# xiph/daala

Measured on NVIDIA H100. Metric: encoder Mpixels/s on 4K YUV420 intra, higher is better.
Workload: dtype int32

## Files before the change

### daala_b200/csrc/kf_engine.cu

```cuda
#include <cuda_runtime.h>
#include <math.h>
#include <stdint.h>
#include <stdio.h>
#include <stdlib.h>
#include <string.h>

#include <algorithm>
#include <cmath>
#include <mutex>
#include <new>
#include <vector>

#include "daala_b200.h"
#include "dering_search.h"
#include "late_skip.h"
#include "mc_batch.h"
#include "gen/coding_order.inc"
#include "pvq_math.cuh"
#include "pvq_warp.cuh"
#include "pvq_common.cuh"

namespace daala_b200 {
namespace kf {

// ... 679 lines not shown
    reinterpret_cast<short4*>(S.res_pack)[r] = pk;
  }
}

struct ItemGeom {
  int blk, band, bn, q, beta, pli, qoff;
  size_t off;
};
__device__ __forceinline__ int band_q(const daala_b200_pvq_params& prm, const daala_b200_kf_frame_quant* fq, int frame,
                                      int pli, int qidx) {
  return fq ? (fq[frame].q0 * fq[frame].pvq_qm_q4[pli][qidx]) >> 4 : (prm.q0 * prm.pvq_qm_q4[pli][qidx]) >> 4;
}
__device__ __forceinline__ ItemGeom item_geom(const daala_b200_pvq_params& prm, uint32_t item,
                                              const daala_b200_kf_frame_quant* fq) {
  ItemGeom g;
  g.blk = (int)(item >> 4);
  g.band = (int)(item & 15);
  const daala_b200_pvq_block b = prm.blocks[g.blk];
  const int bs = b.bs;
  g.pli = b.pli;
  const int start = band_start(g.band);
  g.bn = band_start(g.band + 1) - start;
  g.off = (size_t)b.coef_off + start;
  const int qidx = bs * (bs + 1) + (g.band + 1) - (g.band + 1) / 3;
  int q = band_q(prm, fq, b.frame, g.pli, qidx);
  g.q = q < 1 ? 1 : q;
  g.beta = (prm.use_masking && g.pli == 0 && bs > 0) ? kBeta15 : kBeta1;
  g.qoff = (b.xdec & 1 ? prm.qm_stride : 0) + ((((1 << (2 * bs)) - 1) << 4) / 3) + start;
  return g;
}

template <int kPhase, bool kZeroRef, int kMode, bool kFq = false>
__global__ void __launch_bounds__(128) k_pvq_split(const __grid_constant__ Stage S, int cls, int chunk) {
  const daala_b200_pvq_params& prm = S.prm;
  const int lane = threadIdx.x & 31;
  const int slots = S.sp_slots[cls];
  const int first = chunk * slots;
  const int count = min(S.cnt[S.n_items_at + cls] - first, slots);
  const int vs = cls == 2 ? 128 : 32;
  const int nwarps = (gridDim.x * blockDim.x) >> 5;
  for (int i = (blockIdx.x * blockDim.x + threadIdx.x) >> 5; i < count; i += nwarps) {
    const ItemGeom g = item_geom(prm, S.items[cls][first + i], kFq ? S.fq : nullptr);
    int16_t* vec = S.sp_vec[cls] + (size_t)i * 3 * vs;
    int32_t* lanes = S.sp_lanes[cls] + (size_t)i * kCtxLaneWords * 16;
    int32_t* uni = S.sp_uni[cls] + (size_t)i * kCtxUniWords;
    int16_t* snap = S.sp_snap[cls] + (size_t)i * kMaxEvents * vs;
    const int32_t* r0 = kZeroRef ? nullptr : prm.ref + g.off;
    BandCtx B;
    if (kPhase == 0) {
      band_setup<kMode>(lane, B, prm.in + g.off, r0, g.bn, g.q, g.beta, prm.is_keyframe, g.pli, prm.qm + g.qoff,
                 prm.pvq_norm_lambda, S.rsqrt_tbl);
      band_ctx_store_setup(lane, B, g.bn, vec, vs, lanes, uni);
    } else if (kPhase == 1) {
      band_ctx_load_search(lane, B, g.bn, vec, vs, lanes);
      band_search<kMode>(lane, B, g.bn, snap, vs, S.rsqrt_tbl);
      band_ctx_store_search(lane, B, lanes);
    } else {
      band_ctx_load_finish(lane, B, g.bn, vec, vs, lanes, uni);
      int itheta, max_theta, k;
      double skip_term;
      const int gain = band_finish<kMode>(lane, B, snap, vs, prm.out + g.off, r0, g.bn, g.q, prm.y + g.off, &itheta, &max_theta, &k,
                                   g.beta, &skip_term, prm.is_keyframe, g.pli, prm.qm_inv + g.qoff, prm.pvq_norm_lambda);
      if (lane == 0) {
        const size_t r = (size_t)g.blk * 9 + g.band;
        prm.res_skip_term[r] = skip_term;
        short4 pk;
        pk.x = (short)gain; pk.y = (short)itheta; pk.z = (short)max_theta; pk.w = (short)k;
        reinterpret_cast<short4*>(S.res_pack)[r] = pk;
      }
    }
  }
}

template <int kMode>
// ... 1292 lines not shown
}

static int enqueue_dering_luma(daala_b200_kf* kf, const Dering& D, cudaStream_t s) {
  if (D.search) {
    const int rc = daala_b200_dering_search_enqueue(&D.sb, s);
    if (rc) return rc;
  }
  const int nsb = kf->nhsb * kf->nvsb;
  k_dering_thresholds<<<(kf->F * nsb + 255) / 256, 256, 0, s>>>(
      D.level, D.thr[0], D.thr[1], kf->F * nsb, make_int4(D.tbl[0][0], D.tbl[0][1], D.tbl[0][2], D.tbl[0][3]),
      make_int2(D.tbl[0][4], D.tbl[0][5]), make_int4(D.tbl[1][0], D.tbl[1][1], D.tbl[1][2], D.tbl[1][3]),
      make_int2(D.tbl[1][4], D.tbl[1][5]), D.coded, D.applied, D.frame_tbl, nsb);
  return enqueue_dering_plane(kf, D, 0, s);
}

static int enqueue_dering(daala_b200_kf* kf, const Dering& D, cudaStream_t s) {
  int rc = enqueue_recon(D.frame, 0, 3, s);
  if (!rc) rc = enqueue_dering_luma(kf, D, s);
  for (int p = 1; !rc && p < 3; p++) rc = enqueue_dering_plane(kf, D, p, s);
  return rc;
}

static int dering_launches(const Dering& D, int parts) { return 2 * parts + (D.search ? 5 + 6 + 6 + 1 : 0) + 1 + 3; }

template <bool kZeroRef, bool kFq = false>
static void enqueue_split(daala_b200_kf* kf, const Stage& S, cudaStream_t s) {
  const int grid = kf->sms * 16;
  for (int cls = 2; cls >= 0; cls--) {
    for (int chunk = 0; chunk < S.sp_chunks[cls]; chunk++) {
      if (cls == 2) {
        k_pvq_split<0, kZeroRef, 2, kFq><<<grid, 128, 0, s>>>(S, cls, chunk);
        k_pvq_split<1, kZeroRef, 2><<<grid, 128, 0, s>>>(S, cls, chunk);
        k_pvq_split<2, kZeroRef, 2, kFq><<<grid, 128, 0, s>>>(S, cls, chunk);
      } else {
        k_pvq_split<0, kZeroRef, 1, kFq><<<grid, 128, 0, s>>>(S, cls, chunk);
        k_pvq_split<1, kZeroRef, 1><<<grid, 128, 0, s>>>(S, cls, chunk);
        k_pvq_split<2, kZeroRef, 1, kFq><<<grid, 128, 0, s>>>(S, cls, chunk);
      }
    }
  }
}

template <bool kInter>
static void enqueue_sym(const Sym& Y, int wide, cudaStream_t s) {
  k_sym_rank<<<(Y.F * Y.nsb + 7) / 8, 256, 0, s>>>(Y);
  k_sym_sb_scan<<<1, 1024, 0, s>>>(Y);
  k_sym_place<<<wide, 256, 0, s>>>(Y);
  k_sym_tile_sums<<<Y.ntiles, kTile, 0, s>>>(Y);
  k_sym_tile_scan<<<1, 1024, 0, s>>>(Y);
  k_sym_offsets<<<Y.ntiles, kTile, 0, s>>>(Y);
  k_sym_pack<kInter><<<wide, 256, 0, s>>>(Y);
  k_sym_index<<<1, 256, 0, s>>>(Y);
}

static int kf_enqueue_step_inter(daala_b200_kf* kf, int phases) {
  cudaStream_t s = kf->stream;
  const Lists& L = kf->lists;
  const int wide = kf->sms * 8;
  if (phases & DAALA_B200_KF_LISTS) {
    k_unit_tile_sums<<<L.ntiles, kTile, 0, s>>>(L);
    k_tile_scan<<<1, 1024, 0, s>>>(L);
    k_unit_emit<<<L.ntiles, kTile, 0, s>>>(L);
    k_luma_items<<<wide, 256, 0, s>>>(L);
    k_chroma_items<<<wide, 256, 0, s>>>(L);
    if (kf->cfg.inter_mc) {
      if (cudaMemsetAsync(L.cnt + kMcBadRef, 0, 2 * sizeof(int32_t), s) != cudaSuccess) return (int)cudaGetLastError();
// ... 837 lines not shown
```

### daala_b200/csrc/pvq_warp.cuh

```cuda
#pragma once
#include <math.h>
#include <stdint.h>

#include "pvq_math.cuh"

namespace daala_b200 {
namespace pvq {

constexpr unsigned kFull = 0xffffffffu;
constexpr int kMaxEvents = 14;
constexpr int kRsqrtEntries = 1 << 16;
constexpr int kLogEntries = 1 << 12;
constexpr int kTableDoubles = kRsqrtEntries + kLogEntries;

#ifndef DAALA_B200_PVQ_EXACT_BOUND
#define DAALA_B200_PVQ_EXACT_BOUND 4503599627370496.
#endif
#ifdef DAALA_B200_EMU_STATS
#define PVQ_WARP_STAT(i) (daala_b200_pvq_warp_stats[i]++)
#else
#define PVQ_WARP_STAT(i) ((void)0)
#endif

__device__ __forceinline__ int wsum(int v) { return __reduce_add_sync(kFull, v); }
__device__ __forceinline__ int wmax(int v) { return __reduce_max_sync(kFull, v); }
__device__ __forceinline__ int wmin(int v) { return __reduce_min_sync(kFull, v); }
__device__ __forceinline__ unsigned wmaxu(unsigned v) { return __reduce_max_sync(kFull, v); }
__device__ __forceinline__ long long wsum64(long long s) {
  const int lo = (int)(s & 0xffffff);
  const int hi = (int)(s >> 24);
  return ((long long)wsum(hi) << 24) + wsum(lo);
}
__device__ __forceinline__ double wfetch(double v, int src) {
  int lo = __double2loint(v), hi = __double2hiint(v);
  lo = __shfl_sync(kFull, lo, src);
  hi = __shfl_sync(kFull, hi, src);
  return __hiloint2double(hi, lo);
}
__device__ __forceinline__ int ordered_key(float f) {
  const int b = __float_as_int(f);
  return b ^ ((b >> 31) & 0x7fffffff);
}
__device__ __forceinline__ int pick4(const int (&a)[4], int slot) {
  int v = a[0];
#pragma unroll
  for (int e = 1; e < 4; e++) if (slot == e) v = a[e];
  return v;
}

static __device__ __noinline__ double nl_log(double x) { return log(x); }
static __device__ __noinline__ double nl_acos(double x) { return acos(x); }
static __device__ __noinline__ double nl_sqrt(double x) { return sqrt(x); }
static __device__ __noinline__ double nl_div(double a, double b) { return a / b; }
static __device__ __noinline__ int nl_cos(int32_t x) { return pvq_cos(x); }
static __device__ __noinline__ double nl_rsqrt_small(int i) {
  if (i <= 16) return kRsqrtSmall[i - 1];
  return 1. / sqrt((double)i);
}
__device__ __forceinline__ void pvq_fill_rsqrt_table(double* rsq, int i) {
  if (i < kRsqrtEntries) rsq[i] = i > 0 ? nl_rsqrt_small(i) : 0.;
  else rsq[i] = .9 * (M_LOG2E * nl_log((double)(i > kRsqrtEntries ? i - kRsqrtEntries : 1)));
}
static __device__ __noinline__ long long nl_gain(int32_t acc, int q0, int beta, int bshift) {
  int32_t g;
  const int32_t cg = compute_gain_from_energy(acc, q0, &g, beta, bshift);
  return ((long long)cg << 32) | (uint32_t)g;
}
static __device__ __noinline__ long long nl_theta_k(int32_t qcg, int j, int ts, int noref, int n, int beta) {
  const int32_t qtheta = noref ? 0 : compute_theta(j, ts);
  const int k = compute_k(qcg, j, noref, n, beta);
  return ((long long)qtheta << 32) | (uint32_t)k;
}

__device__ __forceinline__ void householder_apply_warp(int lane, bool big, int (&out)[4], const int (&x)[4],
                                                       const int (&r)[4], int n) {
  int32_t l2r = 0, proj = 0;
#pragma unroll
  for (int e = 0; e < 4; e++) {
    if (e && !big) break;
    if (e * 32 + lane < n) {
      l2r += mul16(r[e], r[e]);
      proj += mul16(r[e], x[e]);
    }
  }
  l2r = wsum(l2r);
  proj = wsum(proj);
  int l2r_shift = (ilog((uint32_t)l2r) - 1) - 14;
  int16_t l2r_norm = (int16_t)vshr_round(l2r, l2r_shift);
  int16_t rcp = rcp16(l2r_norm);
  int proj_shift = (ilog((uint32_t)abs(proj)) - 1) - 14;
  int16_t proj_norm = (int16_t)vshr_round(proj, proj_shift);
  int16_t proj_1 = (int16_t)mul16_q15(proj_norm, rcp);
  int outshift = 14 - proj_shift - 1 + l2r_shift;
  if (outshift > 30) outshift = 30;
#pragma unroll
  for (int e = 0; e < 4; e++) {
    if (e && !big) break;
    int32_t t = mul16(r[e], proj_1);
    t = outshift >= 0 ? shr_round(t, outshift) : shl(t, -outshift);
    out[e] = (int16_t)(x[e] - t);
  }
}

struct SearchVec {
  int xa[4];
  double xx, norm_1, l1_norm;
  double delta_rate;
  int xmax, nn;
};

template <int E>
__device__ __forceinline__ void search_init(int lane, SearchVec& v, const int (&src)[4], int nn) {
  long long sxx = 0;
  int xmax = 0, sl1 = 0;
#pragma unroll
  for (int e = 0; e < E; e++) {
    const int a = e * 32 + lane < nn ? abs(src[e]) : 0;
    v.xa[e] = a;
    sxx += (long long)a * a;
    sl1 += a;
    xmax = a > xmax ? a : xmax;
  }
  v.xx = (double)wsum64(sxx);
  v.xmax = wmax(xmax);
  v.l1_norm = (double)wsum(sl1);
  v.norm_1 = nl_div(1., nl_sqrt(1e-30 + v.xx));
  v.delta_rate = nl_div(3., (double)nn);
  v.nn = nn;
}

__device__ __forceinline__ int search_start(int lane, const SearchVec& v, int (&ya)[4], int k, int prev_k, bool big,
                                            double* xy, double* yy) {
  const int nn = v.nn;
  long long sxy = 0, syy = 0;
  int si = 0;
  if (prev_k > 0 && prev_k <= k) {
#pragma unroll
    for (int e = 0; e < 4; e++) {
      if (e && !big) break;
      if (e * 32 + lane >= nn) ya[e] = 0;
      sxy += (long long)v.xa[e] * ya[e];
      syy += (long long)ya[e] * ya[e];
      si += ya[e];
    }
  } else if (k > 2) {
    const double l1_inv = nl_div(1., v.l1_norm > 1e-100 ? v.l1_norm : 1e-100);
#pragma unroll
    for (int e = 0; e < 4; e++) {
      if (e && !big) break;
      const double tmp = k * (double)v.xa[e] * l1_inv;
      const int f = (int)floor(tmp);
      ya[e] = (e * 32 + lane < nn && f > 0) ? f : 0;
      sxy += (long long)v.xa[e] * ya[e];
      syy += (long long)ya[e] * ya[e];
      si += ya[e];
    }
  } else {
#pragma unroll
    for (int e = 0; e < 4; e++) ya[e] = 0;
    *xy = 0;
    *yy = 0;
    return 0;
  }
  *xy = (double)wsum64(sxy);
  *yy = (double)wsum64(syy);
  return wsum(si);
}

template <int E>
__device__ __forceinline__ void search_event(int lane, const SearchVec& v, int (&ya)[4], int k, int i, double xy,
                                             double yy, double lambda, const double* rsq, double* xy_out,
                                             double* yy_out) {
  const int nn = v.nn;
  const int rdo_pulses = 1 + k / 4;
  double delta_rate = v.delta_rate;
  double accel_rate = 0.;
  if (k == 1) {
    if (nn == 15) {
      accel_rate = -8. / 15;
      delta_rate = 4.5 / 15 - accel_rate;
    } else if (nn == 8) {
      accel_rate = 5.7 / 8;
      delta_rate = 9.3 / 8 - accel_rate;
    }
  }
  for (; i < k; i++) {
    const bool plain = i < k - rdo_pulses;
    bool cont[E];
    double tval[E];
    int total;
    if (plain) {
      const double bound = (xy + v.xmax) * (xy + v.xmax) * (yy + 2. * i + 1.);
      if (bound < DAALA_B200_PVQ_EXACT_BOUND) {
        const float xyf = (float)xy, yyf1 = (float)(yy + 1.);
        unsigned key[E], kmax = 0;
#pragma unroll
        for (int e = 0; e < E; e++) {
          float a = xyf + (float)v.xa[e];
          a *= a;
// ... 62 lines not shown
#pragma unroll
          for (int t = 1; t < E; t++) if (e == t) m = mk[t];
        }
        if (!m) break;
        const int l = __ffs(m) - 1;
        m &= m - 1;
        int sxa = v.xa[0], sya = ya[0];
        double stv = tval[0];
#pragma unroll
        for (int t = 1; t < E; t++) if (e == t) { sxa = v.xa[t]; sya = ya[t]; stv = tval[t]; }
        if (plain) {
          const int xj = __shfl_sync(kFull, sxa, l);
          const int yj = __shfl_sync(kFull, sya, l);
          double a = xy + (double)xj;
          const double b = yy + 2 * yj + 1;
          a *= a;
          if (pos < 0 || a * bb > ba * b) { ba = a; bb = b; pos = e * 32 + l; }
        } else {
          const double t = wfetch(stv, l);
          if (pos < 0 || t > ba) { ba = t; pos = e * 32 + l; }
        }
      }
    }
    const int src = pos & 31, slot = pos >> 5;
    int sx = v.xa[0], sy = ya[0];
#pragma unroll
    for (int e = 1; e < E; e++) if (slot == e) { sx = v.xa[e]; sy = ya[e]; }
    const int px = __shfl_sync(kFull, sx, src);
    const int py = __shfl_sync(kFull, sy, src);
    xy = xy + (double)px;
    yy = yy + 2 * py + 1;
#pragma unroll
    for (int e = 0; e < E; e++) if (e * 32 + lane == pos) ya[e]++;
  }
  *xy_out = xy;
  *yy_out = yy;
}

struct BandCtx {
  int x16[4], r16[4], xr[4];
  int32_t cg, g, gain_offset;
  int icgr, m, s;
  double best_dist, best_cost, skip_dist;
  int c_gain, c_theta, c_ts, c_k, c_cosd, c_alive, c_ev;
  int32_t c_qcg, c_qtheta;
  double c_sinprod, c_lambda, c_rate_ts;
  double e_xy, e_yy, e_xx;
  int e_sum, e_k, e_zero;
};

constexpr int kCtxLaneWords = 24;
constexpr int kCtxUniWords = 16;
constexpr int kSnapEntries = kMaxEvents * kMaxN + 3 * kMaxN + 2 * (kCtxLaneWords * 16 + kCtxUniWords);

#ifdef __CUDACC__
__device__ __forceinline__ void ctx_sync() { __syncwarp(); }
#else
inline void ctx_sync() {}
#endif

__device__ __forceinline__ void ctx_put_d(int32_t* lanes, int w, int lane, double v) {
  lanes[w * 16 + lane] = __double2loint(v);
  lanes[(w + 1) * 16 + lane] = __double2hiint(v);
}
__device__ __forceinline__ double ctx_get_d(const int32_t* lanes, int w, int lane) {
  return __hiloint2double(lanes[(w + 1) * 16 + lane], lanes[w * 16 + lane]);
// ... 78 lines not shown
  B.c_rate_ts = ctx_get_d(lanes, 12, l);
  B.c_ev = on ? lanes[14 * 16 + l] : -1;
  B.e_xy = on ? ctx_get_d(lanes, 15, l) : 0.;
  B.e_yy = on ? ctx_get_d(lanes, 17, l) : 0.;
  B.e_xx = on ? ctx_get_d(lanes, 19, l) : 0.;
  B.e_sum = on ? lanes[21 * 16 + l] : 0;
  B.e_k = on ? lanes[22 * 16 + l] : 0;
  B.e_zero = on ? lanes[23 * 16 + l] : 0;
  B.cg = uni[0]; B.g = uni[1]; B.gain_offset = uni[2]; B.icgr = uni[3]; B.m = uni[4]; B.s = uni[5];
  B.best_dist = __hiloint2double(uni[7], uni[6]);
  B.best_cost = __hiloint2double(uni[9], uni[8]);
  B.skip_dist = __hiloint2double(uni[11], uni[10]);
}

template <int kMode>
__device__ __forceinline__ void band_setup(int lane, BandCtx& B, const int32_t* x0, const int32_t* r0, int n, int q0,
                                           int beta, int is_keyframe, int pli, const int16_t* qm,
                                           double pvq_norm_lambda, const double* rsq) {
  int (&x16)[4] = B.x16; int (&r16)[4] = B.r16; int (&xr)[4] = B.xr;
  int32_t &cg = B.cg, &g = B.g, &gain_offset = B.gain_offset;
  int &icgr = B.icgr, &m = B.m, &s = B.s;
  double &best_dist = B.best_dist, &best_cost = B.best_cost, &skip_dist = B.skip_dist;
  int &c_gain = B.c_gain, &c_theta = B.c_theta, &c_ts = B.c_ts, &c_k = B.c_k, &c_cosd = B.c_cosd, &c_alive = B.c_alive;
  int32_t &c_qcg = B.c_qcg, &c_qtheta = B.c_qtheta;
  double &c_sinprod = B.c_sinprod, &c_lambda = B.c_lambda, &c_rate_ts = B.c_rate_ts;

  const double gain_weight = 1.4;
  const double cgain_1 = 1. / kCgainOne;
  const double cgain_2 = cgain_1 * cgain_1;
  const double theta_scale = (1 << kThetaShift) * 2. / M_PI;
  const double theta_scale_1 = 1. / theta_scale;
  const double trig_1 = 1. / 32768;
  const bool big = kMode == 0 ? n > 32 : kMode == 2;
  int xshift, rshift, r_nonnull = 0;
  {
    int32_t xv[4], rv[4];
    int32_t sx = 0, sr = 0;
#pragma unroll
    for (int e = 0; e < 4; e++) {
      xv[e] = rv[e] = 0;
      if (e && !big) continue;
      const int j = e * 32 + lane;
      if (j < n) {
        xv[e] = x0[j];
        rv[e] = r0 ? r0[j] : 0;
      }
      const int16_t tx = (int16_t)(xv[e] >> 8), tr = (int16_t)(rv[e] >> 8);
      sx += tx * (int32_t)tx;
      sr += tr * (int32_t)tr;
      r_nonnull |= rv[e] != 0;
    }
    sx = wsum(sx);
    sr = wsum(sr);
    r_nonnull = __any_sync(kFull, r_nonnull);
    xshift = 9 + ilog((uint32_t)(n + sx)) / 2 - 15;
    rshift = 9 + ilog((uint32_t)(n + sr)) / 2 - 14;
    if (xshift < 0) xshift = 0;
    if (rshift < 0) rshift = 0;
#pragma unroll
    for (int e = 0; e < 4; e++) {
      x16[e] = r16[e] = xr[e] = 0;
      if (e && !big) continue;
      const int j = e * 32 + lane;
      const int qmv = j < n ? qm[j] : 0;
      x16[e] = (int16_t)shr_round(xv[e] * qmv, kQmShift + xshift);
      r16[e] = (int16_t)shr_round(rv[e] * qmv, kQmShift + rshift);
    }
  }
  long long scorr = 0;
  int32_t accx = 0, accr = 0;
#pragma unroll
  for (int e = 0; e < 4; e++) {
    if (e && !big) break;
    scorr += mul16(x16[e], r16[e]);
    accx += x16[e] * x16[e];
    accr += r16[e] * r16[e];
  }
  double corr = (double)wsum64(scorr);
  accx = wsum(accx);
  accr = wsum(accr);
  int32_t gr, cgr;
  {
    const long long pk = nl_gain(lane & 1 ? accr : accx, q0, beta, lane & 1 ? rshift : xshift);
    const int gl = (int)(uint32_t)pk, cgl = (int)(pk >> 32);
    g = __shfl_sync(kFull, gl, 0);
    cg = __shfl_sync(kFull, cgl, 0);
    gr = __shfl_sync(kFull, gl, 1);
    cgr = __shfl_sync(kFull, cgl, 1);
  }
  const int cfl_enabled = is_keyframe && pli != 0;
  if (cfl_enabled) cgr = kCgainOne;
  icgr = shr_round(cgr, kCgainShift);
  gain_offset = cgr - shl(icgr, kCgainShift);
  best_dist = gain_weight * cg * cg * cgain_2;
  best_cost = best_dist + pvq_norm_lambda * 0.;
  corr = nl_div(corr, 1e-100 + nl_div(g * (double)gr, (double)shl(1, xshift + rshift)));
  corr = corr < 1. ? corr : 1.;
  corr = corr > -1. ? corr : -1.;
  if (is_keyframe) {
    skip_dist = gain_weight * cg * cg * cgain_2;
  } else {
    skip_dist = gain_weight * (cg - cgr) * (cg - cgr) + cgr * (double)cg * (2 - 2 * corr);
    skip_dist *= cgain_2;
    const int32_t scgr = gain_offset > 0 ? gain_offset : 0;
    if (icgr == 0) {
      best_dist = gain_weight * (cg - scgr) * (cg - scgr) + scgr * (double)cg * (2 - 2 * corr);
      best_dist *= cgain_2;
    }
    best_cost = best_dist + pvq_norm_lambda * 0.;
  }
  const double dist0 = best_dist;

  const bool have_ref = r_nonnull && corr > 0;
  int32_t theta = 0;
  m = 0;
  s = 1;
  if (have_ref) {
    theta = round32(theta_scale * nl_acos(corr));
    int key = -1;
#pragma unroll
    for (int e = 0; e < 4; e++) {
      if (e && !big) break;
      const int j = e * 32 + lane;
      const int kk = j < n ? (abs(r16[e]) << 7) | (127 - j) : -1;
      key = kk > key ? kk : key;
    }
    key = wmax(key);
    m = (key >> 7) > 0 ? 127 - (key & 127) : 0;
    const int rm = __shfl_sync(kFull, pick4(r16, m >> 5), m & 31);
    s = rm > 0 ? 1 : -1;
#pragma unroll
    for (int e = 0; e < 4; e++)
      if (e * 32 + lane == m) r16[e] = (int16_t)(r16[e] + shr_round(gr * s, rshift));
    householder_apply_warp(lane, big, xr, x16, r16, n);
#pragma unroll
    for (int e = 0; e < 4; e++) {
      if (e && !big) break;
      const int t1 = __shfl_sync(kFull, xr[e], (lane + 1) & 31);
      const int t2 = e + 1 < 4 ? __shfl_sync(kFull, xr[e + 1 < 4 ? e + 1 : e], 0) : 0;
      const int nxt = lane == 31 ? t2 : t1;
      if (e * 32 + lane >= m) xr[e] = nxt;
    }
  }

  c_gain = 0; c_theta = -1; c_ts = 0; c_k = 0; c_cosd = 0; c_qcg = 0; c_qtheta = 0;
  c_sinprod = 0; c_lambda = 0; c_rate_ts = 0;
  bool c_valid = false;
  {
    const bool wref = lane < 12;
    const bool nref = lane == 12 || lane == 13;
    int i = 0, j = -1;
    if (wref && have_ref) {
      const int gain_bound = (cg - gain_offset) >> kCgainShift;
      i = (gain_bound - 1 > 1 ? gain_bound - 1 : 1) + (lane >> 2);
      c_valid = i <= gain_bound + 1;
      c_qcg = shl(i, kCgainShift) + gain_offset;
    } else if (nref && ((is_keyframe && pli == 0) || corr < .5 || cg < (int32_t)shl(2, kCgainShift))) {
      const int gain_bound = cg >> kCgainShift;
      i = (gain_bound > 1 ? gain_bound : 1) + (lane - 12);
      c_valid = i <= gain_bound + 1;
      c_qcg = shl(i, kCgainShift);
    }
    if (!c_valid) c_qcg = kCgainOne;
    if (wref) {
      c_ts = compute_max_theta(c_qcg, beta);
      int lo = (int)floor(.5 + nl_div(theta * theta_scale_1 * 2, M_PI) * c_ts) - 2;
      int hi = (int)ceil(nl_div(theta * theta_scale_1 * 2, M_PI) * c_ts);
      if (lo < 0) lo = 0;
      if (hi > c_ts - 1) hi = c_ts - 1;
      j = lo + (lane & 3);
// ... 1 lines not shown
    } else {
      c_ts = 0;
    }
    const long long tk = nl_theta_k(c_qcg, j, c_ts, !wref, n, beta);
    c_qtheta = (int32_t)(tk >> 32);
    c_k = (int)(uint32_t)tk;
    c_gain = i;
    c_theta = wref ? j : -1;
    c_cosd = nl_cos(theta - c_qtheta);
    const int sin_q = nl_cos(32768 - c_qtheta), sin_t = nl_cos(32768 - theta);
    double dist = gain_weight * (c_qcg - cg) * (c_qcg - cg);
    double g2 = c_qcg * (double)cg;
    if (wref) {
      const double dist_theta = 2 - 2. * c_cosd * trig_1;
      dist = dist + c_qcg * (double)cg * dist_theta;
      const double sin_theta = sin_t * trig_1;
      c_sinprod = sin_theta * sin_q * trig_1;
      g2 = g2 * c_sinprod;
    }
    dist *= cgain_2;
    g2 = g2 * cgain_2;
    c_alive = c_valid && !(wref ? dist > dist0 + 1.0 * pvq_norm_lambda && c_k != 0 : dist > dist0 && c_k != 0);
    c_lambda = nl_div(pvq_norm_lambda, 1e-30 + g2);
    c_rate_ts = c_ts < kLogEntries ? rsq[kRsqrtEntries + (c_ts > 0 ? c_ts : 1)]
                                   : .9 * (M_LOG2E * nl_log((double)c_ts));
  }
}

template <int kMode>
__device__ __forceinline__ void band_search(int lane, BandCtx& B, int n, int16_t* snap, int snap_stride,
                                            const double* rsq, const int32_t* pre_ev = nullptr,
                                            const int16_t* pre_snap = nullptr) {
  const bool big = kMode == 0 ? n > 32 : kMode == 2;
  const int (&x16)[4] = B.x16; const int (&xr)[4] = B.xr;
  const int &c_k = B.c_k, &c_alive = B.c_alive;
  const double &c_lambda = B.c_lambda;
  int &c_ev = B.c_ev;
  double &e_xy = B.e_xy, &e_yy = B.e_yy, &e_xx = B.e_xx;
  int &e_sum = B.e_sum, &e_k = B.e_k, &e_zero = B.e_zero;
  unsigned alive_w = __ballot_sync(kFull, c_alive && lane < 12);
  unsigned alive_n = __ballot_sync(kFull, c_alive && lane >= 12);
  if (pre_ev) alive_n = 0;

  int ya[4];
#pragma unroll
  for (int e = 0; e < 4; e++) ya[e] = 0;
  SearchVec sv;
  sv.nn = n;
  sv.xx = 0;
  int prev_k = 0, nev = 0;
  c_ev = -1;
  int phase = 0;
  e_xy = 0; e_yy = 0; e_xx = 0; e_sum = 0; e_k = 0; e_zero = 0;
  while (alive_w | alive_n) {
    unsigned grp;
    int kcur, leader;
    const bool noref_ev = alive_w == 0;
    if (!noref_ev) {
      const int key = (alive_w >> lane) & 1 ? (c_k << 4) | lane : 0x7fffffff;
      const int mn = wmin(key);
      kcur = mn >> 4;
      leader = mn & 15;
      grp = __ballot_sync(kFull, ((alive_w >> lane) & 1) && c_k == kcur);
      alive_w &= ~grp;
    } else {
      leader = __ffs(alive_n) - 1;
      grp = 1u << leader;
      alive_n &= ~grp;
      kcur = __shfl_sync(kFull, c_k, leader);
    }
    const int want = noref_ev ? 2 : 1;
    if (phase != want) {
      phase = want;
      prev_k = 0;
      int src[4];
#pragma unroll
      for (int e = 0; e < 4; e++) src[e] = noref_ev ? x16[e] : xr[e];
      if (big) search_init<4>(lane, sv, src, noref_ev ? n : n - 1);
      else search_init<1>(lane, sv, src, noref_ev ? n : n - 1);
    }
    double xy = 0, yy = 0;
    const bool zero_ev = !noref_ev && kcur == 0;
    if (zero_ev) {
#pragma unroll
      for (int e = 0; e < 4; e++) ya[e] = 0;
    } else {
      const double lambda = wfetch(c_lambda, leader);
      const int i = search_start(lane, sv, ya, kcur, prev_k, big, &xy, &yy);
      if (big) search_event<4>(lane, sv, ya, kcur, i, xy, yy, lambda, rsq, &xy, &yy);
      else search_event<1>(lane, sv, ya, kcur, i, xy, yy, lambda, rsq, &xy, &yy);
    }
    prev_k = kcur;
    int sj = 0;
#pragma unroll
    for (int e = 0; e < 4; e++) {
      if (e && !big) break;
      const int j = e * 32 + lane;
      if (j < sv.nn) sj += j * ya[e];
      if (j < n) snap[nev * snap_stride + j] = (int16_t)(j < sv.nn ? ya[e] : 0);
    }
    sj = wsum(sj);
    if (lane == nev) {
      e_xy = xy;
      e_yy = yy;
      e_xx = sv.xx;
      e_sum = sj;
      e_k = kcur;
      e_zero = zero_ev;
    }
    if ((grp >> lane) & 1) c_ev = nev;
    nev++;
  }
  if (pre_ev) {
    const int cev = (lane == 12 || lane == 13) ? pre_ev[lane - 12] : -1;
    const int nimp = wmax(cev) + 1;
    if (cev >= 0) c_ev = nev + cev;
    if (lane >= nev && lane < nev + nimp) {
      const int32_t* r = pre_ev + 2 + (lane - nev) * 9;
      e_xy = __hiloint2double(r[1], r[0]);
      e_yy = __hiloint2double(r[3], r[2]);
      e_xx = __hiloint2double(r[5], r[4]);
      e_sum = r[6];
      e_k = r[7];
      e_zero = r[8];
    }
    for (int ev = 0; ev < nimp; ev++) {
#pragma unroll
      for (int e = 0; e < 4; e++) {
        if (e && !big) break;
        const int j = e * 32 + lane;
        if (j < n) snap[(nev + ev) * snap_stride + j] = pre_snap[ev * n + j];
      }
    }
  }

}

template <int kMode>
__device__ __forceinline__ int band_finish(int lane, const BandCtx& B, const int16_t* snap, int snap_stride, int32_t* out,
                                           const int32_t* r0, int n, int q0, int32_t* yout, int* itheta,
                                           int* max_theta, int* vk, int beta, double* skip_term, int is_keyframe,
                                           int pli, const int16_t* qm_inv, double pvq_norm_lambda) {
  const double gain_weight = 1.4;
  const double cgain_1 = 1. / kCgainOne;
  const double cgain_2 = cgain_1 * cgain_1;
  const double trig_1 = 1. / 32768;
  const bool big = kMode == 0 ? n > 32 : kMode == 2;
  const int cfl_enabled = is_keyframe && pli != 0;
  const int (&x16)[4] = B.x16; const int (&r16)[4] = B.r16; const int (&xr)[4] = B.xr;
  const int32_t cg = B.cg;
  int32_t g = B.g, gain_offset = B.gain_offset;
  const int icgr = B.icgr, m = B.m, s = B.s;
  double best_dist = B.best_dist, best_cost = B.best_cost;
  const double skip_dist = B.skip_dist;
  const int c_gain = B.c_gain, c_theta = B.c_theta, c_ts = B.c_ts, c_k = B.c_k, c_cosd = B.c_cosd, c_ev = B.c_ev;
  const int32_t c_qcg = B.c_qcg, c_qtheta = B.c_qtheta;
  const double c_sinprod = B.c_sinprod, c_rate_ts = B.c_rate_ts;
  const double e_xy = B.e_xy, e_yy = B.e_yy, e_xx = B.e_xx;
  const int e_sum = B.e_sum, e_k = B.e_k, e_zero = B.e_zero;
  int32_t theta = 0;
  double e_cos = 0, e_rate = 0;
  {
    const int kk = e_k > 0 ? e_k : 1;
    const double cd = nl_div(e_xy, 1e-100 + nl_sqrt(e_xx * e_yy));
    const double f = nl_div((double)e_sum, (double)(kk * n));
    const double t = nl_div(nl_log(n * 2 * (1 * f + .025)) * kk, (double)n);
    const double rate = (1 + .4 * f) * n * (M_LOG2E * nl_log(1 + (0 > t ? 0 : t))) + 3;
    e_cos = e_zero ? 0. : cd;
    e_rate = e_k == 0 ? 0. : rate;
  }
  double c_dist = 0, cost = 0;
  {
    const int src = c_ev >= 0 ? c_ev : 0;
    const double cos_dist = wfetch(e_cos, src);
    double rate = wfetch(e_rate, src);
    double dist;
    if (lane >= 12) {
      dist = gain_weight * (c_qcg - cg) * (c_qcg - cg) + c_qcg * (double)cg * (2 - 2 * cos_dist);
    } else {
      if (c_gain > 0 && c_theta >= 0) {
        rate += c_rate_ts;
        if (is_keyframe && pli == 0) rate += 6;
        if (c_gain == icgr) rate -= .5;
      }
      const double dist_theta = 2 - 2. * c_cosd * trig_1 + c_sinprod * (2 - 2 * cos_dist);
      dist = gain_weight * (c_qcg - cg) * (c_qcg - cg) + c_qcg * (double)cg * dist_theta;
    }
    dist *= cgain_2;
    c_dist = dist;
    cost = dist + pvq_norm_lambda * rate;
  }
  int best_lane = -1;
  {
    unsigned rem = __ballot_sync(kFull, c_ev >= 0);
    while (rem) {
      const int key = (rem >> lane) & 1 ? (c_ev << 5) | lane : 0x7fffffff;
      const int l = wmin(key) & 31;
      rem &= ~(1u << l);
      const double cl = wfetch(cost, l);
      if (l >= 12 ? cl <= best_cost : cl < best_cost) {
        best_cost = cl;
        best_lane = l;
      }
    }
  }

  int qg = 0, best_k = 0;
  int noref = is_keyframe ? 1 : 0;
  *itheta = is_keyframe ? -1 : 0;
  *max_theta = 0;
  int ybest[4];
#pragma unroll
  for (int e = 0; e < 4; e++) ybest[e] = 0;
  if (best_lane >= 0) {
    qg = __shfl_sync(kFull, c_gain, best_lane);
    best_k = __shfl_sync(kFull, c_k, best_lane);
    *itheta = __shfl_sync(kFull, c_theta, best_lane);
    *max_theta = __shfl_sync(kFull, c_ts, best_lane);
    theta = __shfl_sync(kFull, c_qtheta, best_lane);
    best_dist = wfetch(c_dist, best_lane);
    noref = best_lane >= 12;
    const int ev = __shfl_sync(kFull, c_ev, best_lane);
#pragma unroll
    for (int e = 0; e < 4; e++) {
      if (e && !big) break;
      const int j = e * 32 + lane;
      const int v = noref ? x16[e] : xr[e];
      const int a = j < n ? snap[ev * snap_stride + j] : 0;
      ybest[e] = j < (noref ? n : n - 1) ? (v < 0 ? -a : a) : 0;
    }
  }
  int skip = 0;
  if (noref) {
    if (qg == 0) skip = 1;
  } else {
    if (!is_keyframe && qg == 0) skip = icgr ? 1 : 2;
    if (qg == icgr && *itheta == 0 && !cfl_enabled) skip = 2;
  }
  int32_t res[4];
  if (skip) {
#pragma unroll
    for (int e = 0; e < 4; e++) res[e] = (skip == 2 && r0 && e * 32 + lane < n) ? r0[e * 32 + lane] : 0;
  } else {
    if (noref) gain_offset = 0;
    g = gain_expand(shl(qg, kCgainShift) + gain_offset, q0, beta);
    const int nn = n - !noref;
    int syy = 0;
#pragma unroll
    for (int e = 0; e < 4; e++) if (e * 32 + lane < nn) syy += ybest[e] * ybest[e];
    const int yy = wsum(syy);
    int gshift = ilog((uint32_t)g) - 14;
    if (gshift < 0) gshift = 0;
    int32_t scale;
    if (yy == 0) {
      scale = 0;
    } else {
      int rsh;
      const int16_t rs = rsqrt32(yy, &rsh);
      scale = vshr_round64(rs * (int64_t)g, rsh + gshift - 16);
    }
    const int qshift = kQmInvShift - gshift;
    int xs[4];
    if (noref) {
#pragma unroll
      for (int e = 0; e < 4; e++) xs[e] = mul16_32_q16(ybest[e], scale);
    } else {
      scale = round32(scale * (1. / 32768) * nl_cos(32768 - theta));
      int f[4];
#pragma unroll
      for (int e = 0; e < 4; e++) f[e] = e * 32 + lane < nn ? (int16_t)mul16_32_q16(ybest[e], scale) : 0;
      const int xm = (int16_t)floor(.5 + -s * (shr_round(g, gshift)) * (1. / 32768) * nl_cos(theta));
#pragma unroll
      for (int e = 0; e < 4; e++) {
        xs[e] = 0;
        if (e && !big) continue;
        const int t1 = __shfl_sync(kFull, f[e], (lane + 31) & 31);
        const int t2 = e > 0 ? __shfl_sync(kFull, f[e > 0 ? e - 1 : 0], 31) : 0;
        const int fprev = lane == 0 ? t2 : t1;
        const int j = e * 32 + lane;
        xs[e] = j < m ? f[e] : (j == m ? xm : fprev);
        if (j >= n) xs[e] = 0;
      }
      householder_apply_warp(lane, big, xs, xs, r16, n);
    }
#pragma unroll
    for (int e = 0; e < 4; e++) {
      const int j = e * 32 + lane;
      res[e] = j < n ? shr_round(xs[e] * qm_inv[j], qshift) : 0;
    }
  }
#pragma unroll
  for (int e = 0; e < 4; e++) {
    const int j = e * 32 + lane;
    if (j < n) {
      out[j] = res[e];
      yout[j] = ybest[e];
    }
  }
  *vk = best_k;
  *skip_term = skip_dist - best_dist;
  if (is_keyframe) return noref ? qg : (qg < icgr ? -2 * (qg - icgr) - 1 : (qg < 2 * icgr ? 2 * (qg - icgr) : qg - 1));
  {
    const int a = qg + 1, b = icgr + 1;
    return noref ? qg - 1 : (a < b ? -2 * (a - b) - 1 : (a < 2 * b ? 2 * (a - b) : a - 1));
  }
}

constexpr int kPreEvWords = 20;
__device__ __forceinline__ void band_noref_export(int lane, const BandCtx& B, int n, const int16_t* snap,
                                                  int snap_stride, int32_t* pre_ev, int16_t* pre_snap) {
  const int cev = (lane == 12 || lane == 13) ? B.c_ev : -1;
  const int nev = wmax(cev) + 1;
  if (lane == 12 || lane == 13) pre_ev[lane - 12] = B.c_ev;
  if (lane < nev) {
    int32_t* r = pre_ev + 2 + lane * 9;
    r[0] = __double2loint(B.e_xy); r[1] = __double2hiint(B.e_xy);
    r[2] = __double2loint(B.e_yy); r[3] = __double2hiint(B.e_yy);
    r[4] = __double2loint(B.e_xx); r[5] = __double2hiint(B.e_xx);
    r[6] = B.e_sum; r[7] = B.e_k; r[8] = B.e_zero;
  }
  for (int ev = 0; ev < nev; ev++)
// ... 36 lines not shown
```

Before: 2432.

## Pack two small PVQ bands per warp using half-warp reductions

```diff
diff --git a/daala_b200/csrc/kf_engine.cu b/daala_b200/csrc/kf_engine.cu
--- a/daala_b200/csrc/kf_engine.cu
+++ b/daala_b200/csrc/kf_engine.cu
@@ -735,14 +735,20 @@
 
 template <int kPhase, bool kZeroRef, int kMode, bool kFq = false>
 __global__ void __launch_bounds__(128) k_pvq_split(const __grid_constant__ Stage S, int cls, int chunk) {
+  constexpr bool kPair = kMode == 3;
   const daala_b200_pvq_params& prm = S.prm;
-  const int lane = threadIdx.x & 31;
+  const int lane = kPair ? threadIdx.x & 15 : threadIdx.x & 31;
   const int slots = S.sp_slots[cls];
   const int first = chunk * slots;
   const int count = min(S.cnt[S.n_items_at + cls] - first, slots);
   const int vs = cls == 2 ? 128 : 32;
   const int nwarps = (gridDim.x * blockDim.x) >> 5;
-  for (int i = (blockIdx.x * blockDim.x + threadIdx.x) >> 5; i < count; i += nwarps) {
+  for (int w = (blockIdx.x * blockDim.x + threadIdx.x) >> 5; (kPair ? 2 * w : w) < count; w += nwarps) {
+    int i = w;
+    if (kPair) {
+      i = 2 * w + ((threadIdx.x >> 4) & 1);
+      if (i >= count) i = 2 * w;
+    }
     const ItemGeom g = item_geom(prm, S.items[cls][first + i], kFq ? S.fq : nullptr);
     int16_t* vec = S.sp_vec[cls] + (size_t)i * 3 * vs;
     int32_t* lanes = S.sp_lanes[cls] + (size_t)i * kCtxLaneWords * 16;
@@ -2101,6 +2107,10 @@
         k_pvq_split<0, kZeroRef, 2, kFq><<<grid, 128, 0, s>>>(S, cls, chunk);
         k_pvq_split<1, kZeroRef, 2><<<grid, 128, 0, s>>>(S, cls, chunk);
         k_pvq_split<2, kZeroRef, 2, kFq><<<grid, 128, 0, s>>>(S, cls, chunk);
+      } else if (cls == 0) {
+        k_pvq_split<0, kZeroRef, 3, kFq><<<grid, 128, 0, s>>>(S, cls, chunk);
+        k_pvq_split<1, kZeroRef, 3><<<grid, 128, 0, s>>>(S, cls, chunk);
+        k_pvq_split<2, kZeroRef, 3, kFq><<<grid, 128, 0, s>>>(S, cls, chunk);
       } else {
         k_pvq_split<0, kZeroRef, 1, kFq><<<grid, 128, 0, s>>>(S, cls, chunk);
         k_pvq_split<1, kZeroRef, 1><<<grid, 128, 0, s>>>(S, cls, chunk);
diff --git a/daala_b200/csrc/pvq_warp.cuh b/daala_b200/csrc/pvq_warp.cuh
--- a/daala_b200/csrc/pvq_warp.cuh
+++ b/daala_b200/csrc/pvq_warp.cuh
@@ -37,6 +37,53 @@
   hi = __shfl_sync(kFull, hi, src);
   return __hiloint2double(hi, lo);
 }
+
+#ifdef __CUDACC__
+__device__ __forceinline__ int half_base() { return threadIdx.x & 16; }
+#else
+inline int half_base() { return simt_emu::cur_lane() & 16; }
+#endif
+template <bool kH> __device__ __forceinline__ int bsum(int v) {
+  if (!kH) return wsum(v);
+  const int hb = half_base();
+  const unsigned lo = (unsigned)__reduce_add_sync(kFull, hb ? 0 : v);
+  const unsigned all = (unsigned)__reduce_add_sync(kFull, v);
+  return (int)(hb ? all - lo : lo);
+}
+template <bool kH> __device__ __forceinline__ int bmax(int v) {
+  if (!kH) return wmax(v);
+  const int hb = half_base();
+  const int lo = __reduce_max_sync(kFull, hb ? (int)0x80000000 : v);
+  const int hi = __reduce_max_sync(kFull, hb ? v : (int)0x80000000);
+  return hb ? hi : lo;
+}
+template <bool kH> __device__ __forceinline__ int bmin(int v) {
+  if (!kH) return wmin(v);
+  const int hb = half_base();
+  const int lo = __reduce_min_sync(kFull, hb ? 0x7fffffff : v);
+  const int hi = __reduce_min_sync(kFull, hb ? v : 0x7fffffff);
+  return hb ? hi : lo;
+}
+template <bool kH> __device__ __forceinline__ long long bsum64(long long s) {
+  if (!kH) return wsum64(s);
+  const int lo = (int)(s & 0xffffff);
+  const int hi = (int)(s >> 24);
+  return ((long long)bsum<true>(hi) << 24) + bsum<true>(lo);
+}
+template <bool kH> __device__ __forceinline__ unsigned bballot(bool p) {
+  const unsigned b = __ballot_sync(kFull, p);
+  return kH ? (b >> half_base()) & 0xffffu : b;
+}
+template <bool kH> __device__ __forceinline__ bool bany(bool p) {
+  return kH ? bballot<true>(p) != 0 : __any_sync(kFull, p) != 0;
+}
+template <bool kH> __device__ __forceinline__ int bshfl(int v, int src) {
+  return __shfl_sync(kFull, v, kH ? half_base() | src : src);
+}
+template <bool kH> __device__ __forceinline__ double bfetch(double v, int src) {
+  return wfetch(v, kH ? half_base() | src : src);
+}
+
 __device__ __forceinline__ int ordered_key(float f) {
   const int b = __float_as_int(f);
   return b ^ ((b >> 31) & 0x7fffffff);
@@ -72,6 +119,7 @@
   return ((long long)qtheta << 32) | (uint32_t)k;
 }
 
+template <bool kH = false>
 __device__ __forceinline__ void householder_apply_warp(int lane, bool big, int (&out)[4], const int (&x)[4],
                                                        const int (&r)[4], int n) {
   int32_t l2r = 0, proj = 0;
@@ -83,8 +131,8 @@
       proj += mul16(r[e], x[e]);
     }
   }
-  l2r = wsum(l2r);
-  proj = wsum(proj);
+  l2r = bsum<kH>(l2r);
+  proj = bsum<kH>(proj);
   int l2r_shift = (ilog((uint32_t)l2r) - 1) - 14;
   int16_t l2r_norm = (int16_t)vshr_round(l2r, l2r_shift);
   int16_t rcp = rcp16(l2r_norm);
@@ -109,7 +157,7 @@
   int xmax, nn;
 };
 
-template <int E>
+template <int E, bool kH = false>
 __device__ __forceinline__ void search_init(int lane, SearchVec& v, const int (&src)[4], int nn) {
   long long sxx = 0;
   int xmax = 0, sl1 = 0;
@@ -121,20 +169,22 @@
     sl1 += a;
     xmax = a > xmax ? a : xmax;
   }
-  v.xx = (double)wsum64(sxx);
-  v.xmax = wmax(xmax);
-  v.l1_norm = (double)wsum(sl1);
+  v.xx = (double)bsum64<kH>(sxx);
+  v.xmax = bmax<kH>(xmax);
+  v.l1_norm = (double)bsum<kH>(sl1);
   v.norm_1 = nl_div(1., nl_sqrt(1e-30 + v.xx));
   v.delta_rate = nl_div(3., (double)nn);
   v.nn = nn;
 }
 
+template <bool kH = false>
 __device__ __forceinline__ int search_start(int lane, const SearchVec& v, int (&ya)[4], int k, int prev_k, bool big,
-                                            double* xy, double* yy) {
+                                            double* xy, double* yy, bool run = true) {
   const int nn = v.nn;
   long long sxy = 0, syy = 0;
   int si = 0;
-  if (prev_k > 0 && prev_k <= k) {
+  if (!run) {
+  } else if (prev_k > 0 && prev_k <= k) {
 #pragma unroll
     for (int e = 0; e < 4; e++) {
       if (e && !big) break;
@@ -158,13 +208,15 @@
   } else {
 #pragma unroll
     for (int e = 0; e < 4; e++) ya[e] = 0;
-    *xy = 0;
-    *yy = 0;
-    return 0;
-  }
-  *xy = (double)wsum64(sxy);
-  *yy = (double)wsum64(syy);
-  return wsum(si);
+    if (!kH) {
+      *xy = 0;
+      *yy = 0;
+      return 0;
+    }
+  }
+  *xy = (double)bsum64<kH>(sxy);
+  *yy = (double)bsum64<kH>(syy);
+  return bsum<kH>(si);
 }
 
 template <int E>
@@ -293,6 +345,100 @@
     yy = yy + 2 * py + 1;
 #pragma unroll
     for (int e = 0; e < E; e++) if (e * 32 + lane == pos) ya[e]++;
+  }
+  *xy_out = xy;
+  *yy_out = yy;
+}
+
+__device__ __forceinline__ void search_event_half(int lane, const SearchVec& v, int (&ya)[4], int k, int i, double xy,
+                                                  double yy, double lambda, const double* rsq, double* xy_out,
+                                                  double* yy_out) {
+  const int hb = half_base();
+  const int nn = v.nn;
+  const int rdo_pulses = 1 + k / 4;
+  double delta_rate = v.delta_rate;
+  double accel_rate = 0.;
+  if (k == 1) {
+    if (nn == 15) {
+      accel_rate = -8. / 15;
+      delta_rate = 4.5 / 15 - accel_rate;
+    } else if (nn == 8) {
+      accel_rate = 5.7 / 8;
+      delta_rate = 9.3 / 8 - accel_rate;
+    }
+  }
+  const int rem = k - i;
+  const int rem_other = __shfl_sync(kFull, rem, (hb ^ 16) | lane);
+  const int iters = rem > rem_other ? rem : rem_other;
+  for (int it = 0; it < iters; it++, i++) {
+    const bool act = i < k;
+    const bool plain = i < k - rdo_pulses;
+    const bool in = act && lane < nn;
+    int key;
+    bool lit = false;
+    double tval = 0;
+    if (plain) {
+      const double bound = (xy + v.xmax) * (xy + v.xmax) * (yy + 2. * i + 1.);
+      lit = !(bound < DAALA_B200_PVQ_EXACT_BOUND);
+      float a = (float)xy + (float)v.xa[0];
+      a *= a;
+      const float b = (float)(yy + 1.) + (float)(2 * ya[0]);
+      key = in ? __float_as_int(__fdividef(a, b)) : (int)0x80000000;
+    } else {
+      const int iyy = yy < 1e9 ? (int)yy : 1000000000;
+      const int arg = iyy + 2 * ya[0] + 1;
+      const double ryy = arg < kRsqrtEntries ? rsq[arg] : nl_rsqrt_small((int)(yy + 2 * ya[0] + 1));
+      double t = xy + (double)v.xa[0];
+      t = 2 * t * v.norm_1 * ryy - lambda * lane * (delta_rate + lane * accel_rate);
+      tval = t;
+      key = in ? ordered_key((float)t) : (int)0x80000000;
+    }
+    const int mx = bmax<true>(key);
+    bool cont;
+    if (plain) {
+      const int thr = mx > 64 ? mx - 64 : 0;
+      cont = in && (lit || key >= thr);
+    } else {
+      cont = in && key == mx;
+    }
+    const unsigned bal = __ballot_sync(kFull, cont);
+    const unsigned mine = (bal >> hb) & 0xffffu;
+    const int total = __popc(mine);
+    if (act) {
+      if (lit) PVQ_WARP_STAT(3);
+      PVQ_WARP_STAT(total == 1 ? 0 : plain ? 1 : 2);
+    }
+    int pos = total == 1 ? __ffs(mine) - 1 : -1;
+    unsigned sm = 0;
+    if (__popc(bal & 0xffffu) > 1) sm |= bal & 0xffffu;
+    if (__popc(bal >> 16) > 1) sm |= bal & 0xffff0000u;
+    double ba = 0, bb = 1;
+    while (sm) {
+      const unsigned my = (sm >> hb) & 0xffffu;
+      const int l = my ? __ffs(my) - 1 : 0;
+      const unsigned lo = sm & 0xffffu, hi = sm & 0xffff0000u;
+      sm = (lo & (lo - 1)) | (hi & (hi - 1));
+      const int w0 = __shfl_sync(kFull, plain ? v.xa[0] : __double2loint(tval), hb | l);
+      const int w1 = __shfl_sync(kFull, plain ? ya[0] : __double2hiint(tval), hb | l);
+      if (!my) continue;
+      if (plain) {
+        double a = xy + (double)w0;
+        const double b = yy + 2 * w1 + 1;
+        a *= a;
+        if (pos < 0 || a * bb > ba * b) { ba = a; bb = b; pos = l; }
+      } else {
+        const double t = __hiloint2double(w1, w0);
+        if (pos < 0 || t > ba) { ba = t; pos = l; }
+      }
+    }
+    const int src = pos >= 0 ? pos : 0;
+    const int px = __shfl_sync(kFull, v.xa[0], hb | src);
+    const int py = __shfl_sync(kFull, ya[0], hb | src);
+    if (act) {
+      xy = xy + (double)px;
+      yy = yy + 2 * py + 1;
+      if (lane == pos) ya[0]++;
+    }
   }
   *xy_out = xy;
   *yy_out = yy;
@@ -437,6 +583,7 @@
   const double theta_scale_1 = 1. / theta_scale;
   const double trig_1 = 1. / 32768;
   const bool big = kMode == 0 ? n > 32 : kMode == 2;
+  constexpr bool kH = kMode == 3;
   int xshift, rshift, r_nonnull = 0;
   {
     int32_t xv[4], rv[4];
@@ -455,9 +602,9 @@
       sr += tr * (int32_t)tr;
       r_nonnull |= rv[e] != 0;
     }
-    sx = wsum(sx);
-    sr = wsum(sr);
-    r_nonnull = __any_sync(kFull, r_nonnull);
+    sx = bsum<kH>(sx);
+    sr = bsum<kH>(sr);
+    r_nonnull = kH ? (int)bany<true>(r_nonnull) : __any_sync(kFull, r_nonnull);
     xshift = 9 + ilog((uint32_t)(n + sx)) / 2 - 15;
     rshift = 9 + ilog((uint32_t)(n + sr)) / 2 - 14;
     if (xshift < 0) xshift = 0;
@@ -481,17 +628,17 @@
     accx += x16[e] * x16[e];
     accr += r16[e] * r16[e];
   }
-  double corr = (double)wsum64(scorr);
-  accx = wsum(accx);
-  accr = wsum(accr);
+  double corr = (double)bsum64<kH>(scorr);
+  accx = bsum<kH>(accx);
+  accr = bsum<kH>(accr);
   int32_t gr, cgr;
   {
     const long long pk = nl_gain(lane & 1 ? accr : accx, q0, beta, lane & 1 ? rshift : xshift);
     const int gl = (int)(uint32_t)pk, cgl = (int)(pk >> 32);
-    g = __shfl_sync(kFull, gl, 0);
-    cg = __shfl_sync(kFull, cgl, 0);
-    gr = __shfl_sync(kFull, gl, 1);
-    cgr = __shfl_sync(kFull, cgl, 1);
+    g = bshfl<kH>(gl, 0);
+    cg = bshfl<kH>(cgl, 0);
+    gr = bshfl<kH>(gl, 1);
+    cgr = bshfl<kH>(cgl, 1);
   }
   const int cfl_enabled = is_keyframe && pli != 0;
   if (cfl_enabled) cgr = kCgainOne;
@@ -520,8 +667,9 @@
   int32_t theta = 0;
   m = 0;
   s = 1;
-  if (have_ref) {
-    theta = round32(theta_scale * nl_acos(corr));
+  if (kH ? __any_sync(kFull, have_ref) != 0 : have_ref) {
+    const bool own = !kH || have_ref;
+    if (own) theta = round32(theta_scale * nl_acos(corr));
     int key = -1;
 #pragma unroll
     for (int e = 0; e < 4; e++) {
@@ -530,17 +678,26 @@
       const int kk = j < n ? (abs(r16[e]) << 7) | (127 - j) : -1;
       key = kk > key ? kk : key;
     }
-    key = wmax(key);
-    m = (key >> 7) > 0 ? 127 - (key & 127) : 0;
-    const int rm = __shfl_sync(kFull, pick4(r16, m >> 5), m & 31);
-    s = rm > 0 ? 1 : -1;
+    key = bmax<kH>(key);
+    const int mm = (key >> 7) > 0 ? 127 - (key & 127) : 0;
+    const int rm = bshfl<kH>(pick4(r16, mm >> 5), mm & 31);
+    if (own) {
+      m = mm;
+      s = rm > 0 ? 1 : -1;
+    }
 #pragma unroll
     for (int e = 0; e < 4; e++)
-      if (e * 32 + lane == m) r16[e] = (int16_t)(r16[e] + shr_round(gr * s, rshift));
-    householder_apply_warp(lane, big, xr, x16, r16, n);
+      if (own && e * 32 + lane == m) r16[e] = (int16_t)(r16[e] + shr_round(gr * s, rshift));
+    householder_apply_warp<kH>(lane, big, xr, x16, r16, n);
 #pragma unroll
     for (int e = 0; e < 4; e++) {
       if (e && !big) break;
+      if (kH) {
+        const int t1 = bshfl<true>(xr[e], (lane + 1) & 15);
+        if (lane >= m) xr[e] = lane == 15 ? 0 : t1;
+        if (!own) xr[e] = 0;
+        continue;
+      }
       const int t1 = __shfl_sync(kFull, xr[e], (lane + 1) & 31);
       const int t2 = e + 1 < 4 ? __shfl_sync(kFull, xr[e + 1 < 4 ? e + 1 : e], 0) : 0;
       const int nxt = lane == 31 ? t2 : t1;
@@ -608,6 +765,7 @@
                                             const double* rsq, const int32_t* pre_ev = nullptr,
                                             const int16_t* pre_snap = nullptr) {
   const bool big = kMode == 0 ? n > 32 : kMode == 2;
+  constexpr bool kH = kMode == 3;
   const int (&x16)[4] = B.x16; const int (&xr)[4] = B.xr;
   const int &c_k = B.c_k, &c_alive = B.c_alive;
   const double &c_lambda = B.c_lambda;
@@ -628,11 +786,31 @@
   c_ev = -1;
   int phase = 0;
   e_xy = 0; e_yy = 0; e_xx = 0; e_sum = 0; e_k = 0; e_zero = 0;
+  const int hb = kH ? half_base() : 0;
   while (alive_w | alive_n) {
     unsigned grp;
     int kcur, leader;
-    const bool noref_ev = alive_w == 0;
-    if (!noref_ev) {
+    bool act = true;
+    bool noref_ev;
+    if (kH) {
+      const unsigned mw = (alive_w >> hb) & 0xffffu, mr = (alive_n >> hb) & 0xffffu;
+      act = (mw | mr) != 0;
+      noref_ev = mw == 0;
+      const int key = (mw >> lane) & 1 ? (c_k << 4) | lane : 0x7fffffff;
+      const int mn = bmin<true>(key);
+      leader = noref_ev ? (mr ? __ffs(mr) - 1 : 0) : mn & 15;
+      kcur = bshfl<true>(c_k, leader);
+      const unsigned gw = __ballot_sync(kFull, ((mw >> lane) & 1) && c_k == kcur);
+      unsigned nr = 0;
+#pragma unroll
+      for (int h = 0; h < 32; h += 16) {
+        const unsigned r = alive_n & (0xffffu << h);
+        if (!(alive_w & (0xffffu << h))) nr |= r & (0u - r);
+      }
+      alive_w &= ~gw;
+      alive_n &= ~nr;
+      grp = !act ? 0u : noref_ev ? 1u << leader : (gw >> hb) & 0xffffu;
+    } else if (!(noref_ev = alive_w == 0)) {
       const int key = (alive_w >> lane) & 1 ? (c_k << 4) | lane : 0x7fffffff;
       const int mn = wmin(key);
       kcur = mn >> 4;
@@ -646,7 +824,21 @@
       kcur = __shfl_sync(kFull, c_k, leader);
     }
     const int want = noref_ev ? 2 : 1;
-    if (phase != want) {
+    if (kH) {
+      const bool need = act && phase != want;
+      if (__any_sync(kFull, need)) {
+        int src[4];
+#pragma unroll
+        for (int e = 0; e < 4; e++) src[e] = noref_ev ? x16[e] : xr[e];
+        SearchVec t;
+        search_init<1, true>(lane, t, src, noref_ev ? n : n - 1);
+        if (need) {
+          sv = t;
+          phase = want;
+          prev_k = 0;
+        }
+      }
+    } else if (phase != want) {
       phase = want;
       prev_k = 0;
       int src[4];
@@ -657,7 +849,15 @@
     }
     double xy = 0, yy = 0;
     const bool zero_ev = !noref_ev && kcur == 0;
-    if (zero_ev) {
+    if (kH) {
+      const bool run = act && !zero_ev;
+      if (act && zero_ev) ya[0] = 0;
+      if (__any_sync(kFull, run)) {
+        const double lambda = bfetch<true>(c_lambda, leader);
+        const int i = search_start<true>(lane, sv, ya, kcur, prev_k, false, &xy, &yy, run);
+        search_event_half(lane, sv, ya, run ? kcur : i, i, xy, yy, lambda, rsq, &xy, &yy);
+      }
+    } else if (zero_ev) {
 #pragma unroll
       for (int e = 0; e < 4; e++) ya[e] = 0;
     } else {
@@ -666,17 +866,17 @@
       if (big) search_event<4>(lane, sv, ya, kcur, i, xy, yy, lambda, rsq, &xy, &yy);
       else search_event<1>(lane, sv, ya, kcur, i, xy, yy, lambda, rsq, &xy, &yy);
     }
-    prev_k = kcur;
+    if (act) prev_k = kcur;
     int sj = 0;
 #pragma unroll
     for (int e = 0; e < 4; e++) {
       if (e && !big) break;
       const int j = e * 32 + lane;
       if (j < sv.nn) sj += j * ya[e];
-      if (j < n) snap[nev * snap_stride + j] = (int16_t)(j < sv.nn ? ya[e] : 0);
-    }
-    sj = wsum(sj);
-    if (lane == nev) {
+      if (act && j < n) snap[nev * snap_stride + j] = (int16_t)(j < sv.nn ? ya[e] : 0);
+    }
+    sj = bsum<kH>(sj);
+    if (act && lane == nev) {
       e_xy = xy;
       e_yy = yy;
       e_xx = sv.xx;
@@ -685,9 +885,9 @@
       e_zero = zero_ev;
     }
     if ((grp >> lane) & 1) c_ev = nev;
-    nev++;
-  }
-  if (pre_ev) {
+    if (act) nev++;
+  }
+  if (!kH && pre_ev) {
     const int cev = (lane == 12 || lane == 13) ? pre_ev[lane - 12] : -1;
     const int nimp = wmax(cev) + 1;
     if (cev >= 0) c_ev = nev + cev;
@@ -722,6 +922,7 @@
   const double cgain_2 = cgain_1 * cgain_1;
   const double trig_1 = 1. / 32768;
   const bool big = kMode == 0 ? n > 32 : kMode == 2;
+  constexpr bool kH = kMode == 3;
   const int cfl_enabled = is_keyframe && pli != 0;
   const int (&x16)[4] = B.x16; const int (&r16)[4] = B.r16; const int (&xr)[4] = B.xr;
   const int32_t cg = B.cg;
@@ -748,8 +949,8 @@
   double c_dist = 0, cost = 0;
   {
     const int src = c_ev >= 0 ? c_ev : 0;
-    const double cos_dist = wfetch(e_cos, src);
-    double rate = wfetch(e_rate, src);
+    const double cos_dist = bfetch<kH>(e_cos, src);
+    double rate = bfetch<kH>(e_rate, src);
     double dist;
     if (lane >= 12) {
       dist = gain_weight * (c_qcg - cg) * (c_qcg - cg) + c_qcg * (double)cg * (2 - 2 * cos_dist);
@@ -767,7 +968,22 @@
     cost = dist + pvq_norm_lambda * rate;
   }
   int best_lane = -1;
-  {
+  if (kH) {
+    const unsigned both = __ballot_sync(kFull, c_ev >= 0);
+    const int lo = __popc(both & 0xffffu), hi = __popc(both >> 16);
+    unsigned rem = (both >> half_base()) & 0xffffu;
+    for (int it = lo > hi ? lo : hi; it > 0; it--) {
+      const int key = (rem >> lane) & 1 ? (c_ev << 5) | lane : 0x7fffffff;
+      const int l = bmin<true>(key) & 15;
+      const double cl = bfetch<true>(cost, l);
+      if (!rem) continue;
+      rem &= ~(1u << l);
+      if (l >= 12 ? cl <= best_cost : cl < best_cost) {
+        best_cost = cl;
+        best_lane = l;
+      }
+    }
+  } else {
     unsigned rem = __ballot_sync(kFull, c_ev >= 0);
     while (rem) {
       const int key = (rem >> lane) & 1 ? (c_ev << 5) | lane : 0x7fffffff;
@@ -788,7 +1004,26 @@
   int ybest[4];
 #pragma unroll
   for (int e = 0; e < 4; e++) ybest[e] = 0;
-  if (best_lane >= 0) {
+  if (kH) {
+    if (__any_sync(kFull, best_lane >= 0)) {
+      const int bl = best_lane & 15;
+      const int t_qg = bshfl<true>(c_gain, bl), t_k = bshfl<true>(c_k, bl), t_it = bshfl<true>(c_theta, bl);
+      const int t_mt = bshfl<true>(c_ts, bl), t_th = bshfl<true>(c_qtheta, bl), ev = bshfl<true>(c_ev, bl);
+      const double t_dist = bfetch<true>(c_dist, bl);
+      if (best_lane >= 0) {
+        qg = t_qg;
+        best_k = t_k;
+        *itheta = t_it;
+        *max_theta = t_mt;
+        theta = t_th;
+        best_dist = t_dist;
+        noref = best_lane >= 12;
+        const int v = noref ? x16[0] : xr[0];
+        const int a = lane < n ? snap[ev * snap_stride + lane] : 0;
+        ybest[0] = lane < (noref ? n : n - 1) ? (v < 0 ? -a : a) : 0;
+      }
+    }
+  } else if (best_lane >= 0) {
     qg = __shfl_sync(kFull, c_gain, best_lane);
     best_k = __shfl_sync(kFull, c_k, best_lane);
     *itheta = __shfl_sync(kFull, c_theta, best_lane);
@@ -814,7 +1049,7 @@
     if (qg == icgr && *itheta == 0 && !cfl_enabled) skip = 2;
   }
   int32_t res[4];
-  if (skip) {
+  if (skip && !kH) {
 #pragma unroll
     for (int e = 0; e < 4; e++) res[e] = (skip == 2 && r0 && e * 32 + lane < n) ? r0[e * 32 + lane] : 0;
   } else {
@@ -824,7 +1059,7 @@
     int syy = 0;
 #pragma unroll
     for (int e = 0; e < 4; e++) if (e * 32 + lane < nn) syy += ybest[e] * ybest[e];
-    const int yy = wsum(syy);
+    const int yy = bsum<kH>(syy);
     int gshift = ilog((uint32_t)g) - 14;
     if (gshift < 0) gshift = 0;
     int32_t scale;
@@ -837,10 +1072,11 @@
     }
     const int qshift = kQmInvShift - gshift;
     int xs[4];
-    if (noref) {
+    if (noref && !kH) {
 #pragma unroll
       for (int e = 0; e < 4; e++) xs[e] = mul16_32_q16(ybest[e], scale);
     } else {
+      const int32_t scale_noref = scale;
       scale = round32(scale * (1. / 32768) * nl_cos(32768 - theta));
       int f[4];
 #pragma unroll
@@ -850,19 +1086,21 @@
       for (int e = 0; e < 4; e++) {
         xs[e] = 0;
         if (e && !big) continue;
-        const int t1 = __shfl_sync(kFull, f[e], (lane + 31) & 31);
+        const int t1 = kH ? bshfl<true>(f[e], (lane + 15) & 15) : __shfl_sync(kFull, f[e], (lane + 31) & 31);
         const int t2 = e > 0 ? __shfl_sync(kFull, f[e > 0 ? e - 1 : 0], 31) : 0;
         const int fprev = lane == 0 ? t2 : t1;
         const int j = e * 32 + lane;
         xs[e] = j < m ? f[e] : (j == m ? xm : fprev);
         if (j >= n) xs[e] = 0;
       }
-      householder_apply_warp(lane, big, xs, xs, r16, n);
+      householder_apply_warp<kH>(lane, big, xs, xs, r16, n);
+      if (kH && noref) xs[0] = mul16_32_q16(ybest[0], scale_noref);
     }
 #pragma unroll
     for (int e = 0; e < 4; e++) {
       const int j = e * 32 + lane;
       res[e] = j < n ? shr_round(xs[e] * qm_inv[j], qshift) : 0;
+      if (kH && skip) res[e] = (skip == 2 && r0 && j < n) ? r0[j] : 0;
     }
   }
 #pragma unroll
```

Result: faster. 2492, median of 6 (+2.5%).
